# MachinePerceptionLab/Attentive_DFPrior

Measured on AMD Instinct MI355X. Metric: rendered rays/sec (64 samples/ray), Replica room0, higher is better.
Workload: dtype f32 via f16x3 split (3 f16 MFMA products per f32 product: 22-bit products, f32 accumulate); 1 GPU; room0 640x480 render_img, 64 spp (48+16), synthetic box room, seed-0 random decoders, grids at the REFERENCE init (N(0,.01), high N(0,1e-4)); stage color, ray_batch_size 100000 (per-batch far clamp, rendered as one call with a depth maximum per 100 000-ray segment), ONE frame per step; samples_per_ray=64

## Files before the change

attentive_dfprior_amd/csrc/adfp_decode_g.h:

```cpp
#pragma once
#include "adfp_decode_h.h"

__host__ __device__ constexpr int unit16(int k) { return 16 * ((k & 7) >> 2) + 4 * (k >> 3) + (k & 3); }

template <int CDIM, int NOUT>
struct DecLayoutG {
    using F = DecLayout<CDIM, NOUT>;
    static constexpr int KG_E = 3;
    static constexpr int KG_C = CDIM / 32;
    __host__ __device__ static constexpr int kg(int i) { return i == 0 ? KG_E : (i == 3 ? KG_E + 1 : 1); }
    static constexpr int P_BM = 0;
    __host__ __device__ static constexpr int layer_words(int i) { return kg(i) * 1024 + 32 + KG_C * 1024 + 32; }
    __host__ __device__ static constexpr int P_WP(int i) {
        int o = 384;
        for (int k = 0; k < i; ++k) o += layer_words(k);
        return o;
    }
    __host__ __device__ static constexpr int P_BP(int i) { return P_WP(i) + kg(i) * 1024; }
    __host__ __device__ static constexpr int P_WC(int i) { return P_BP(i) + 32; }
    __host__ __device__ static constexpr int P_BC(int i) { return P_WC(i) + KG_C * 1024; }
    static constexpr int P_WO = P_WP(5);
    static constexpr int P_BO = P_WO + NOUT * 32;
    static constexpr int P_FLAG = P_BO + 4;
    static constexpr int NFLAG = (((P_FLAG + 511) / 256) + 3) & ~3;
// ... 42 lines not shown

template <int CDIM, int NOUT>
ADFP_DEV void pack_decoder_g_block(int blk, const float* __restrict__ flat, unsigned* __restrict__ packed, int* __restrict__ status, int bit) {
    using L = DecLayoutG<CDIM, NOUT>;
    const int t = blk * 256 + (int)threadIdx.x;
    HSrc s{0, -1, -1};
    float a = 0.f, b = 0.f;
    if (t < L::P_FLAG) {
        s = dec_g_src<CDIM, NOUT>(t);
        a = s.s0 < 0 ? 0.f : flat[s.s0]; b = s.s1 < 0 ? 0.f : flat[s.s1];
    }
    pack_block_flag(!(fmaxf(fabsf(a), fabsf(b)) < 65504.0f), packed + L::P_FLAG + blk, status, bit);
    if (t >= L::P_FLAG) return;
    if (s.kind == 0) { packed[t] = s.s0 < 0 ? 0u : __float_as_uint(a); return; }
    a = f16_clamp(a); b = f16_clamp(b);
    const float ah = f16_hi_part(a), bh = f16_hi_part(b);
    _Float16 x, y;
    if (s.kind == 1) { x = (_Float16)ah; y = (_Float16)bh; }
    else { x = (_Float16)(a - ah); y = (_Float16)(b - bh); }
    packed[t] = (unsigned)__builtin_bit_cast(unsigned short, x) | ((unsigned)__builtin_bit_cast(unsigned short, y) << 16);
}
template <int CDIM, int NOUT>
__global__ void k_pack_decoder_g(const float* __restrict__ flat, unsigned* __restrict__ packed, int* __restrict__ status, int bit) { pack_decoder_g_block<CDIM, NOUT>((int)blockIdx.x, flat, packed, status, bit); }

typedef float f32x4g __attribute__((ext_vector_type(4)));

ADFP_DEV void swap_halves(float& x, float& y) {
    const auto r = __builtin_amdgcn_permlane32_swap(__float_as_uint(x), __float_as_uint(y), false, false);
    x = __uint_as_float(r[0]); y = __uint_as_float(r[1]);
}

template <int NG>
ADFP_DEV void mfma_chain_g(f32x4g acc[2][2], const unsigned* __restrict__ w, const f16x8 (*xh)[2], const f16x8 (*xl)[2]) {
#pragma unroll
    for (int kg = 0; kg < NG; ++kg) {
#pragma unroll
        for (int ob = 0; ob < 2; ++ob) {
            const f16x8 ah = __builtin_bit_cast(f16x8, *(const u32x4*)(w + kg * 1024 + ob * 512));
            const f16x8 al = __builtin_bit_cast(f16x8, *(const u32x4*)(w + kg * 1024 + ob * 512 + 256));
#pragma unroll
            for (int pb = 0; pb < 2; ++pb) {
                acc[ob][pb] = __builtin_amdgcn_mfma_f32_16x16x32_f16(ah, xh[kg][pb], acc[ob][pb], 0, 0, 0);
                acc[ob][pb] = __builtin_amdgcn_mfma_f32_16x16x32_f16(ah, xl[kg][pb], acc[ob][pb], 0, 0, 0);
                acc[ob][pb] = __builtin_amdgcn_mfma_f32_16x16x32_f16(al, xh[kg][pb], acc[ob][pb], 0, 0, 0);
            }
        }
    }
    __builtin_amdgcn_sched_barrier(0);
}

ADFP_DEV void row_store(float* p, const f32x4 v) {
    *(f32x4*)p = v;
}
template <int CDIM, int NOUT, int TRAIN = 0>
ADFP_DEV void decode_net_g(const unsigned* __restrict__ ldsu, const GridDev& grid, const GridDev& grid1, const float pn[3], const float (*pf)[3],
                           int lane, float& amax, float (*out)[NOUT], unsigned* __restrict__ mw, float* srow0, unsigned rowbits) {
    using L = DecLayoutG<CDIM, NOUT>;
    using ST = DecStage<CDIM>;
    const int g = lane >> 4;
    float* srow[2] = {nullptr, nullptr};
    if constexpr (TRAIN) {
        srow[0] = (rowbits & 1u) ? srow0 : nullptr;
        srow[1] = (rowbits & 2u) ? srow0 + 16 * ST::NXM : nullptr;
    }
    const unsigned* wl = ldsu + 4 * lane;
    const float* b4 = (const float*)ldsu + 4 * g;
    const float* brow = (const float*)ldsu + 32 * g;
    f16x8 ch[L::KG_C][2], cl[L::KG_C][2];
#pragma unroll
    for (int kc = 0; kc < L::KG_C; ++kc) {
        float c[16];
        gather16(kc == 0 ? grid : grid1, pn, g & 1, c);
        float x[8] = {c[0], c[1], c[2], c[3], c[8], c[9], c[10], c[11]};
        float y[8] = {c[4], c[5], c[6], c[7], c[12], c[13], c[14], c[15]};
#pragma unroll
        for (int s = 0; s < 8; ++s) swap_halves(x[s], y[s]);
        if constexpr (TRAIN) {
            static_assert(!TRAIN || CDIM == 32, "training rows: 32-channel decoders");
            if (srow[0]) { row_store(srow[0] + ST::xm(ST::SC) + 4 * g, f32x4{x[0], x[1], x[2], x[3]}); row_store(srow[0] + ST::xm(ST::SC) + 16 + 4 * g, f32x4{x[4], x[5], x[6], x[7]}); }
            if (srow[1]) { row_store(srow[1] + ST::xm(ST::SC) + 4 * g, f32x4{y[0], y[1], y[2], y[3]}); row_store(srow[1] + ST::xm(ST::SC) + 16 + 4 * g, f32x4{y[4], y[5], y[6], y[7]}); }
        }
        split8(x, ch[kc][0], cl[kc][0], amax);
        split8(y, ch[kc][1], cl[kc][1], amax);
    }
    f16x8 eh[L::KG_E][2], el[L::KG_E][2];
#pragma unroll
    for (int kg = 0; kg < L::KG_E; ++kg) {
        float e0[8], e1[8];
#pragma unroll
        for (int j = 0; j < 8; ++j) {
            const f32x4 bm = *(const f32x4*)(brow + L::P_BM + (32 * kg + j) * 4);
            e0[j] = adfp_sinf(fmaf(pf[0][2], bm.z, fmaf(pf[0][1], bm.y, pf[0][0] * bm.x)));
            e1[j] = adfp_sinf(fmaf(pf[1][2], bm.z, fmaf(pf[1][1], bm.y, pf[1][0] * bm.x)));
        }
        split8<false>(e0, eh[kg][0], el[kg][0], amax);
        split8<false>(e1, eh[kg][1], el[kg][1], amax);
    }
    __builtin_amdgcn_sched_barrier(0);
    f32x4g acc[2][2];
    f16x8 hh[1][2], hl[1][2];
    unsigned mk[3] = {0u, 0u, 0u};
#pragma unroll
    for (int i = 0; i < 5; ++i) {
#pragma unroll
        for (int ob = 0; ob < 2; ++ob) { const f32x4 t = *(const f32x4*)(b4 + L::P_BP(i) + 16 * ob); acc[ob][0] = t; acc[ob][1] = t; }
        if (i == 0) mfma_chain_g<L::KG_E>(acc, wl + L::P_WP(0), eh, el);
        else if (i == 3) {
            mfma_chain_g<L::KG_E>(acc, wl + L::P_WP(3), eh, el);
            mfma_chain_g<1>(acc, wl + L::P_WP(3) + L::KG_E * 1024, hh, hl);
        } else mfma_chain_g<1>(acc, wl + L::P_WP(i), hh, hl);
#pragma unroll
        for (int ob = 0; ob < 2; ++ob) {
            const f32x4 t = *(const f32x4*)(b4 + L::P_BC(i) + 16 * ob);
#pragma unroll
            for (int pb = 0; pb < 2; ++pb)
#pragma unroll
                for (int r = 0; r < 4; ++r) {
                    const float v = relu_f(acc[ob][pb][r]);
                    if constexpr (TRAIN) mk[i >> 1] = __builtin_amdgcn_alignbit(mk[i >> 1], 0u - __float_as_uint(v), 31);
                    acc[ob][pb][r] = v + t[r];
                }
        }
        mfma_chain_g<L::KG_C>(acc, wl + L::P_WC(i), ch, cl);
        if constexpr (TRAIN) {
#pragma unroll
            for (int pb = 0; pb < 2; ++pb) if (srow[pb]) {
                row_store(srow[pb] + ST::xm(ST::SH(i)) + 4 * g, f32x4{acc[0][pb][0], acc[0][pb][1], acc[0][pb][2], acc[0][pb][3]});
                row_store(srow[pb] + ST::xm(ST::SH(i)) + 16 + 4 * g, f32x4{acc[1][pb][0], acc[1][pb][1], acc[1][pb][2], acc[1][pb][3]});
            }
        }
        if (i < 4) {
#pragma unroll
            for (int pb = 0; pb < 2; ++pb) {
                const float t[8] = {acc[0][pb][0], acc[0][pb][1], acc[0][pb][2], acc[0][pb][3],
                                    acc[1][pb][0], acc[1][pb][1], acc[1][pb][2], acc[1][pb][3]};
                split8(t, hh[0][pb], hl[0][pb], amax);
            }
        }
    }
#pragma unroll
    for (int o = 0; o < NOUT; ++o) {
        const f32x4 w0 = *(const f32x4*)(b4 + L::P_WO + 32 * o), w1 = *(const f32x4*)(b4 + L::P_WO + 32 * o + 16);
#pragma unroll
        for (int pb = 0; pb < 2; ++pb) {
            float s = 0.f;
#pragma unroll
            for (int r = 0; r < 4; ++r) s = fmaf(acc[0][pb][r], w0[r], s);
#pragma unroll
            for (int r = 0; r < 4; ++r) s = fmaf(acc[1][pb][r], w1[r], s);
            s += __shfl_xor(s, 16);
            s += __shfl_xor(s, 32);
            out[pb][o] = s + ((const float*)ldsu)[L::P_BO + o];
        }
    }
    if constexpr (TRAIN) {
        const int sh = 4 * (g >> 1);
        unsigned wpb[2][3];
#pragma unroll
        for (int pb = 0; pb < 2; ++pb) {
            unsigned f[5];
#pragma unroll
            for (int i = 0; i < 5; ++i) {
                const unsigned m16 = (i == 4 || (i & 1)) ? (mk[i >> 1] & 0xFFFFu) : (mk[i >> 1] >> 16);
                const unsigned n0 = (m16 >> (12 - 4 * pb)) & 0xFu, n1 = (m16 >> (4 - 4 * pb)) & 0xFu;
                f[i] = (n0 << (12 - sh)) | (n1 << (4 - sh));
            }
            wpb[pb][0] = f[0] | (f[1] << 16); wpb[pb][1] = f[2] | (f[3] << 16); wpb[pb][2] = f[4];
        }
#pragma unroll
        for (int k = 0; k < 3; ++k) {
            const auto r = __builtin_amdgcn_permlane32_swap(wpb[0][k], wpb[1][k], false, false);
            mw[k] = r[0] | r[1];
        }
    }
}

template <int NT>
__global__ __launch_bounds__(NT, NT / 256) void k_decode_lc16(DecodeLCArgs a) {
    using LL = DecLayoutG<32, 1>;
    using LC = DecLayoutG<32, 4>;
    __shared__ __attribute__((aligned(16))) unsigned lds_all[LL::P_TOTAL + LC::P_TOTAL];
    __shared__ int s_next;
    __shared__ unsigned long long s_ring[ADFP_POOL_RING];
    unsigned* lds_low = lds_all;
    unsigned* lds_col = lds_all + LL::P_TOTAL;
    image_to_lds<NT, LL::P_TOTAL / 4>(lds_low, a.packed_low);
    image_to_lds<NT, LC::P_TOTAL / 4>(lds_col, a.packed_color);
    if (threadIdx.x == 0) s_next = NT / 64;
    if (threadIdx.x < ADFP_POOL_RING) s_ring[threadIdx.x] = 0ull;
    __syncthreads();
    const int lane = threadIdx.x & 63, n = lane & 15, g = lane >> 4;
    const int count = a.P.n;
    const int ntiles = (count + 31) >> 5;
    const TilePlan plan = tile_plan(ntiles, (int)gridDim.x, NT / 64, a.pool != nullptr);
    float amax_low = image_out_of_range<LL::P_FLAG, LL::NFLAG>(lds_low) ? INFINITY : 0.f;
    float amax_col = image_out_of_range<LC::P_FLAG, LC::NFLAG>(lds_col) ? INFINITY : 0.f;
    for (int j = threadIdx.x >> 6, tile; (tile = claim_tile_pool<NT / 64>(j, &s_next, s_ring, plan, ntiles, a.pool, a.status)) >= 0;) {
        const int idx = tile * 32 + 16 * (g >> 1) + n;
        const bool valid = idx < count;
        const int q = valid ? idx : 0;
        float pn[3], pf[2][3];
        bool pnan, keep_occ;
        {
            double pt[3];
            load_point(a.P, q, pt);
            normalize3(a.nb, pt, pn);
            const float f0 = (float)pt[0], f1 = (float)pt[1], f2 = (float)pt[2];
            pnan = (pt[0] != pt[0]) | (pt[1] != pt[1]) | (pt[2] != pt[2]);
            const unsigned f = a.flags ? a.flags[q] : 0u;
            keep_occ = (f & ADFP_F_BAND) || in_bound(pt, a.b) || !a.apply_bound;
            pf[0][0] = f0; pf[0][1] = f1; pf[0][2] = f2; pf[1][0] = f0; pf[1][1] = f1; pf[1][2] = f2;
        }
#pragma unroll
        for (int k = 0; k < 3; ++k) swap_halves(pf[0][k], pf[1][k]);
        float occ[2][1], rgb[2][4];
        int off_low = 0, off_col = LL::P_TOTAL;
        asm volatile("" : "+v"(off_low), "+v"(off_col));
        decode_net_g<32, 1>(lds_all + off_low, a.g_low, a.g_low, pn, pf, lane, amax_low, occ, nullptr, nullptr, 0u);
        asm volatile("" : "+v"(pn[0]), "+v"(pn[1]), "+v"(pn[2]), "+v"(occ[0][0]), "+v"(occ[1][0]));
        __builtin_amdgcn_sched_barrier(0);
        decode_net_g<32, 4>(lds_all + off_col, a.g_color, a.g_color, pn, pf, lane, amax_col, rgb, nullptr, nullptr, 0u);
        if (valid && (g & 1) == 0) {
            const int pb = g >> 1;
            const float nanv = __builtin_nanf("");
            const float o = pnan ? nanv : (keep_occ ? (pb ? occ[1][0] : occ[0][0]) : 100.f);
            const f32x4 c4 = pb ? f32x4{rgb[1][0], rgb[1][1], rgb[1][2], o} : f32x4{rgb[0][0], rgb[0][1], rgb[0][2], o};
            *(f32x4*)(a.raw + 4ll * q) = pnan ? f32x4{nanv, nanv, nanv, o} : c4;
            if (a.write_w) a.w[q] = 1.f;
        }
    }
    report_range(a.status, amax_low, ADFP_STATUS_F16_RANGE_LOW, a.call_flag);
    report_range(a.status, amax_col, ADFP_STATUS_F16_RANGE_COLOR, a.call_flag);
}

struct DecodeLCTrainArgs {
    DecodeLCArgs f;
    unsigned* masks_low; unsigned* masks_color;
    float* act_low; float* act_color;
    int split_networks;
};
template <int NT, bool SPLIT = false>
__global__ __launch_bounds__(NT, NT / 256) void k_decode_lc16_train(DecodeLCTrainArgs t) {
    const DecodeLCArgs& a = t.f;
    using LL = DecLayoutG<32, 1>;
    using LC = DecLayoutG<32, 4>;
    using ST = DecStage<32>;
    __shared__ __attribute__((aligned(16))) unsigned lds_all[LL::P_TOTAL + LC::P_TOTAL];
    __shared__ int s_next;
    unsigned* lds_low = lds_all;
    unsigned* lds_col = lds_all + LL::P_TOTAL;
    image_to_lds<NT, LL::P_TOTAL / 4>(lds_low, a.packed_low);
    image_to_lds<NT, LC::P_TOTAL / 4>(lds_col, a.packed_color);
    if (threadIdx.x == 0) s_next = NT / 64;
    __syncthreads();
    const int lane = threadIdx.x & 63, n = lane & 15, g = lane >> 4;
    const int count = a.P.n;
    const int ntiles = (count + 31) >> 5;
    float amax_low = image_out_of_range<LL::P_FLAG, LL::NFLAG>(lds_low) ? INFINITY : 0.f;
    float amax_col = image_out_of_range<LC::P_FLAG, LC::NFLAG>(lds_col) ? INFINITY : 0.f;
    constexpr bool split = SPLIT;
    const int njobs = split ? 2 * ntiles : ntiles;
    for (int j = threadIdx.x >> 6, job; (job = claim_tile<NT / 64>(j, &s_next, njobs)) >= 0;) {
// ... 8 lines not shown
            double pt[3];
            load_point(a.P, q, pt);
            normalize3(a.nb, pt, pn);
            pnan = (pt[0] != pt[0]) | (pt[1] != pt[1]) | (pt[2] != pt[2]);
            const float f0 = pnan ? 0.f : (float)pt[0], f1 = pnan ? 0.f : (float)pt[1], f2 = pnan ? 0.f : (float)pt[2];
            const unsigned f = a.flags ? a.flags[q] : 0u;
            keep_occ = (f & ADFP_F_BAND) || in_bound(pt, a.b) || !a.apply_bound;
            pf[0][0] = f0; pf[0][1] = f1; pf[0][2] = f2; pf[1][0] = f0; pf[1][1] = f1; pf[1][2] = f2;
        }
#pragma unroll
        for (int k = 0; k < 3; ++k) swap_halves(pf[0][k], pf[1][k]);
        const int i0 = tile * 32 + n;
        const unsigned rowbits = (i0 < count ? 1u : 0u) | (i0 + 16 < count ? 2u : 0u);
        float occ[2][1], rgb[2][4];
        unsigned mw[3];
        int off_low = 0, off_col = LL::P_TOTAL;
        asm volatile("" : "+v"(off_low), "+v"(off_col));
        if constexpr (split) {
            occ[0][0] = 0.f; occ[1][0] = 0.f;
#pragma unroll
            for (int k = 0; k < 4; ++k) { rgb[0][k] = 0.f; rgb[1][k] = 0.f; }
        }
        if (do_low) {
            decode_net_g<32, 1, 1>(lds_all + off_low, a.g_low, a.g_low, pn, pf, lane, amax_low, occ, mw, t.act_low + (long long)i0 * ST::NXM, t.act_low ? rowbits : 0u);
            if (valid) { unsigned* mrow = t.masks_low + ((long long)q * 2 + (g & 1)) * 3; mrow[0] = mw[0]; mrow[1] = mw[1]; mrow[2] = mw[2]; }
        }
        asm volatile("" : "+v"(pn[0]), "+v"(pn[1]), "+v"(pn[2]), "+v"(occ[0][0]), "+v"(occ[1][0]));
        __builtin_amdgcn_sched_barrier(0);
        if (do_col) {
            decode_net_g<32, 4, 1>(lds_all + off_col, a.g_color, a.g_color, pn, pf, lane, amax_col, rgb, mw, t.act_color + (long long)i0 * ST::NXM, t.act_color ? rowbits : 0u);
            if (valid) { unsigned* mrow = t.masks_color + ((long long)q * 2 + (g & 1)) * 3; mrow[0] = mw[0]; mrow[1] = mw[1]; mrow[2] = mw[2]; }
        }
        if (valid && (g & 1) == 0) {
            const int pb = g >> 1;
            const float nanv = __builtin_nanf("");
            const float o = pnan ? nanv : (keep_occ ? (pb ? occ[1][0] : occ[0][0]) : 100.f);
            const f32x4 c4 = pb ? f32x4{rgb[1][0], rgb[1][1], rgb[1][2], o} : f32x4{rgb[0][0], rgb[0][1], rgb[0][2], o};
            const f32x4 row = pnan ? f32x4{nanv, nanv, nanv, o} : c4;
            if (!split) {
                *(f32x4*)(a.raw + 4ll * q) = row;
                if (a.write_w) a.w[q] = 1.f;
            } else if (do_low) {
                a.raw[4ll * q + 3] = row.w;
                if (a.write_w) a.w[q] = 1.f;
            } else {
                a.raw[4ll * q] = row.x; a.raw[4ll * q + 1] = row.y; a.raw[4ll * q + 2] = row.z;
            }
        }
    }
    report_range(a.status, amax_low, ADFP_STATUS_F16_RANGE_LOW, a.call_flag);
    report_range(a.status, amax_col, ADFP_STATUS_F16_RANGE_COLOR, a.call_flag);
}

template <int NT>
__global__ __launch_bounds__(NT, NT / 256) void k_decode_high_g(DecodeArgs a) {
    using L = DecLayoutG<64, 1>;
    __shared__ __attribute__((aligned(16))) unsigned ldsu[L::P_TOTAL];
    __shared__ int s_next;
    __shared__ unsigned long long s_ring[ADFP_POOL_RING];
    image_to_lds<NT, L::P_TOTAL / 4>(ldsu, a.packed);
    if (threadIdx.x == 0) s_next = NT / 64;
    if (threadIdx.x < ADFP_POOL_RING) s_ring[threadIdx.x] = 0ull;
    __syncthreads();
    const int lane = threadIdx.x & 63, n = lane & 15, g = lane >> 4;
    const int count = *a.count_ptr;
    const int ntiles = (count + 31) >> 5;
    const TilePlan plan = tile_plan(ntiles, (int)gridDim.x, NT / 64, a.pool != nullptr);
    float amax = image_out_of_range<L::P_FLAG, L::NFLAG>(ldsu) ? INFINITY : 0.f;
    for (int j = threadIdx.x >> 6, tile; (tile = claim_tile_pool<NT / 64>(j, &s_next, s_ring, plan, ntiles, a.pool, a.status)) >= 0;) {
        const int idx = tile * 32 + 16 * (g >> 1) + n;
        const bool valid = idx < count;
        const int q = a.list[valid ? idx : 0];
        float pn[3], pf[2][3];
        bool pnan;
        const float low_occ = (a.single || !valid) ? 0.f : a.raw[4ll * q + 3];
        {
            double pt[3];
            load_point(a.P, q, pt);
            normalize3(a.nb, pt, pn);
            const float f0 = (float)pt[0], f1 = (float)pt[1], f2 = (float)pt[2];
            pnan = (pt[0] != pt[0]) | (pt[1] != pt[1]) | (pt[2] != pt[2]);
            pf[0][0] = f0; pf[0][1] = f1; pf[0][2] = f2; pf[1][0] = f0; pf[1][1] = f1; pf[1][2] = f2;
        }
#pragma unroll
        for (int k = 0; k < 3; ++k) swap_halves(pf[0][k], pf[1][k]);
        float out[2][1];
        decode_net_g<64, 1>(ldsu, a.g0, a.g1, pn, pf, lane, amax, out, nullptr, nullptr, 0u);
        if (valid && (g & 1) == 0) {
            const float o = g >> 1 ? out[1][0] : out[0][0];
            const float v = pnan ? __builtin_nanf("") : o;
            a.att_occ[idx] = a.single ? v : v + low_occ;
        }
    }
    report_range(a.status, amax, ADFP_STATUS_F16_RANGE_HIGH, a.call_flag);
}

struct AttLayoutG {
    using F = AttLayout;
    static constexpr int P_A0 = 0;
    static constexpr int P_W1 = 256;
    static constexpr int P_B1 = P_W1 + 4 * 2 * 1024;
    static constexpr int P_W2 = P_B1 + 128;
    static constexpr int P_B2 = P_W2 + 4 * 4 * 1024;
    static constexpr int P_W3 = P_B2 + 128;
    static constexpr int P_B3 = P_W3 + 2 * 4 * 1024;
    static constexpr int P_WO = P_B3 + 64;
    static constexpr int P_BO = P_WO + 128;
    static constexpr int P_FLAG = P_BO + 4;
    static constexpr int NFLAG = (((P_FLAG + 511) / 256) + 3) & ~3;
    static constexpr int P_TOTAL = P_FLAG + NFLAG;
    static_assert((P_TOTAL + 255) / 256 <= NFLAG, "one flag word per pack block");
};

__device__ HSrc att_g_src(int t) {
    using L = AttLayoutG;
    using F = AttLayout;
    if (t < L::P_W1) {
        const int row = t >> 2, c = t & 3;
        const int u = (row & ~31) + unit16(row & 31);
        return HSrc{0, c < 2 ? F::F_W0 + u * 2 + c : (c == 2 ? F::F_B0 + u : -1), -1};
    }
    auto chain = [](int u, int ngrp, int base, int ld) {
        const int blk = u / (ngrp * 1024), v = u % (ngrp * 1024);
        const int grp = v >> 10, ob = (v >> 9) & 1, part = (v >> 8) & 1, g = (v >> 6) & 3, row = 32 * blk + 16 * ob + ((v >> 2) & 15), jp = (v & 3) * 2;
        return HSrc{1 + part, base + row * ld + 32 * grp + unit16(8 * g + jp), base + row * ld + 32 * grp + unit16(8 * g + jp + 1)};
    };
    if (t < L::P_B1) return chain(t - L::P_W1, 2, F::F_W1, 64);
    if (t < L::P_W2) return HSrc{0, F::F_B1 + (t - L::P_B1), -1};
    if (t < L::P_B2) return chain(t - L::P_W2, 4, F::F_W2, 128);
    if (t < L::P_W3) return HSrc{0, F::F_B2 + (t - L::P_B2), -1};
    if (t < L::P_B3) return chain(t - L::P_W3, 4, F::F_W3, 128);
    if (t < L::P_WO) return HSrc{0, F::F_B3 + (t - L::P_B3), -1};
    if (t < L::P_BO) return HSrc{0, F::F_WO + (t - L::P_WO), -1};
    const int o = t - L::P_BO;
    return HSrc{0, o < 2 ? F::F_BO + o : -1, -1};
}

ADFP_DEV void pack_attention_g_block(int blk, const float* __restrict__ flat, unsigned* __restrict__ packed, int* __restrict__ status) {
    using L = AttLayoutG;
    const int t = blk * 256 + (int)threadIdx.x;
    HSrc s{0, -1, -1};
    float a = 0.f, b = 0.f;
    if (t < L::P_FLAG) {
        s = att_g_src(t);
// ... 125 lines not shown
```

attentive_dfprior_amd/csrc/adfp_device.h:

```cpp
#pragma once
#include <hip/hip_runtime.h>
#include <stdint.h>
#include "adfp.h"

typedef float f32x16 __attribute__((ext_vector_type(16)));
typedef float f32x4 __attribute__((ext_vector_type(4)));

#define ADFP_DEV __device__ __forceinline__

#define ADFP_F_INBOUND 1u
#define ADFP_F_BAND    2u

struct NormDev {
    double lo[3];
    double inv[3];
};

struct GridDev { const float* data; int Z, Y, X; float fZ1, fY1, fX1; };
struct TsdfDev { const float* data; int Z, Y, X; long long sZ, sY, sX; const float* cb; };

struct PtsDev {
    int mode;
    int S;
    int n;
    const void* pts;
    const float* ro;
    const float* rd;
    const double* z;
};

ADFP_DEV void load_point(const PtsDev& P, int q, double p[3]) {
    if (P.mode == ADFP_PTS_RAYS) {
        const int r = (int)((unsigned)q / (unsigned)P.S);
        const double z = P.z[q];
#pragma unroll
        for (int k = 0; k < 3; ++k)
            p[k] = __dadd_rn((double)P.ro[3 * r + k], __dmul_rn((double)P.rd[3 * r + k], z));
    } else if (P.mode == ADFP_PTS_F64) {
        const double* s = (const double*)P.pts + 3ll * q;
        p[0] = s[0]; p[1] = s[1]; p[2] = s[2];
    } else {
        const float* s = (const float*)P.pts + 3ll * q;
        p[0] = (double)s[0]; p[1] = (double)s[1]; p[2] = (double)s[2];
    }
}

ADFP_DEV bool in_bound(const double p[3], const double b[6]) {
    return (p[0] < b[1]) & (p[0] > b[0]) & (p[1] < b[3]) & (p[1] > b[2]) & (p[2] < b[5]) & (p[2] > b[4]);
}

ADFP_DEV void normalize3(const NormDev& nb, const double p[3], float pn[3]) {
#pragma unroll
    for (int k = 0; k < 3; ++k) pn[k] = (float)(((p[k] - nb.lo[k]) * nb.inv[k]) * 2.0 - 1.0);
}

ADFP_DEV void tri_axis(float pn, int size, int& i0, int& i1, float& w0, float& w1) {
    float c = ((pn + 1.f) / 2.f) * (float)(size - 1);
    c = fminf(fmaxf(c, 0.f), (float)(size - 1));
    const float f = floorf(c);
    i0 = (int)f;
    w1 = c - f;
    w0 = (f + 1.f) - c;
    i1 = i0 + 1;
    if (i1 > size - 1) { i1 = size - 1; w1 = 0.f; }
}

typedef float f32x2_u __attribute__((ext_vector_type(2), aligned(4)));
ADFP_DEV float trilerp_scalar(const TsdfDev& t, const float pn[3]) {
    int x0, x1, y0, y1, z0, z1; float wx0, wx1, wy0, wy1, wz0, wz1;
    tri_axis(pn[0], t.X, x0, x1, wx0, wx1);
    tri_axis(pn[1], t.Y, y0, y1, wy0, wy1);
    tri_axis(pn[2], t.Z, z0, z1, wz0, wz1);
    const float* d = t.data;
    const long long ox0 = x0 * t.sX, ox1 = x1 * t.sX, oy0 = y0 * t.sY, oy1 = y1 * t.sY;
    float v000, v001, v010, v011, v100, v101, v110, v111;
    if (t.sZ == 1 && t.Z >= 2) {
        const int zb = z0 < t.Z - 1 ? z0 : t.Z - 2;
        const bool lo = z0 == zb;
        const f32x2_u p00 = *(const f32x2_u*)(d + zb + oy0 + ox0);
        const f32x2_u p01 = *(const f32x2_u*)(d + zb + oy0 + ox1);
        const f32x2_u p10 = *(const f32x2_u*)(d + zb + oy1 + ox0);
        const f32x2_u p11 = *(const f32x2_u*)(d + zb + oy1 + ox1);
        v000 = lo ? p00.x : p00.y; v100 = p00.y;
        v001 = lo ? p01.x : p01.y; v101 = p01.y;
        v010 = lo ? p10.x : p10.y; v110 = p10.y;
        v011 = lo ? p11.x : p11.y; v111 = p11.y;
    } else {
        const long long oz0 = z0 * t.sZ, oz1 = z1 * t.sZ;
        v000 = d[oz0 + oy0 + ox0]; v001 = d[oz0 + oy0 + ox1];
        v010 = d[oz0 + oy1 + ox0]; v011 = d[oz0 + oy1 + ox1];
// ... 411 lines not shown
```

attentive_dfprior_amd/csrc/adfp_kernels.hip:

```cpp
#include "adfp_device.h"
#include <math.h>
#include <string.h>
#include <stdio.h>
#include <stdlib.h>

#define ADFP_CHECK_LAUNCH()                         \
    do {                                            \
        hipError_t e_ = hipGetLastError();          \
        if (e_ != hipSuccess) return (int)e_;       \
    } while (0)

__global__ __launch_bounds__(256) void k_zero(unsigned* __restrict__ p, long long n_words) {
    const long long n4 = n_words >> 2;
    const long long stride = (long long)gridDim.x * 256;
    if ((((unsigned long long)p) & 15ull) == 0) {
        for (long long i = (long long)blockIdx.x * 256 + threadIdx.x; i < n4; i += stride) ((uint4*)p)[i] = uint4{0u, 0u, 0u, 0u};
        for (long long i = (n4 << 2) + (long long)blockIdx.x * 256 + threadIdx.x; i < n_words; i += stride) p[i] = 0u;
    } else {
        for (long long i = (long long)blockIdx.x * 256 + threadIdx.x; i < n_words; i += stride) p[i] = 0u;
    }
}
#define ZERO_MULTI 8
struct ZeroJobs { unsigned* p[ZERO_MULTI]; long long words[ZERO_MULTI]; unsigned first_block[ZERO_MULTI + 1]; int n; };
__device__ inline void zero_multi_block(const ZeroJobs& z, unsigned blk) {
// ... 1579 lines not shown
    PtsDev P; int rc = make_pts(pts, &P); if (rc) return rc;
    adfp_scene sc; memset(&sc, 0, sizeof(sc));
    sc.tsdf = *tsdf;
    for (int k = 0; k < 3; ++k) { sc.tsdf_bnds[k][0] = tsdf_bnds[k][0]; sc.tsdf_bnds[k][1] = tsdf_bnds[k][1]; sc.bound[k][0] = 0; sc.bound[k][1] = 1; }
    return launch_tsdf(&sc, P, nullptr, nullptr, nullptr, nullptr, nullptr, out, (hipStream_t)stream);
}

static int decode_grid(int ntiles, int waves_per_wg, int wg_per_cu) {
    int g = (ntiles + waves_per_wg - 1) / waves_per_wg;
    const int cap = num_cu() * wg_per_cu;
    if (g > cap) g = cap;
    return g < 1 ? 1 : g;
}

static int eval_points_impl(const adfp_scene* sc, const PtsDev& P, int stage, int apply_bound, float* raw, float* w, Workspace& ws_in, hipStream_t st,
                            const adfp_train_state* state = nullptr, bool ws_counter_is_zero = false) {
    if (P.n == 0) return 0;
    Workspace ws = ws_in;
    if (state) {
        ws.flags = state->flags; ws.list = state->list; ws.counter = state->counter;
        ws.att_occ = state->att_occ; ws.att_u = state->att_u;
    }
    hipError_t e;
    const bool fuse = stage != ADFP_STAGE_LOW;
    if (stage != ADFP_STAGE_COLOR) {
        e = zero_async(raw, (size_t)P.n * 16, st);
        if (e != hipSuccess) return (int)e;
    }
    const bool any_h = sc->h_low || (fuse && (sc->h_high || sc->h_att)) || (stage == ADFP_STAGE_COLOR && sc->h_color);
    int* call_flag = (any_h && ws.counter) ? ws.counter + 8 : nullptr;
    if ((fuse || any_h || state) && ws.counter && !ws_counter_is_zero) {
        e = zero_async(ws.counter, 64, st);
        if (e != hipSuccess) return (int)e;
    }
    if (fuse) {
        int rc = launch_tsdf(sc, P, ws.flags, ws.list, ws.att_u, nullptr, ws.counter, nullptr, st);
        if (rc) return rc;
    }
    DecodeArgs a;
    a.P = P; a.nb = make_norm(sc->bound); fill_bound(a.b, sc->bound);
    a.list = nullptr; a.count_ptr = nullptr; a.flags = fuse ? ws.flags : nullptr;
    a.raw = raw; a.w = w; a.att_occ = nullptr; a.write_w = 1; a.apply_bound = apply_bound;
    a.status = sc->status; a.masks = nullptr; a.act = nullptr; a.single = 0; a.call_flag = call_flag;
    const int ntiles = (P.n + 31) / 32;
    const bool fused_lc = stage == ADFP_STAGE_COLOR && !state && sc->h_low && sc->h_color;
    if (fused_lc) {
        DecodeLCArgs f;
        f.P = P; f.nb = a.nb; fill_bound(f.b, sc->bound);
        f.g_low = make_grid(sc->low); f.g_color = make_grid(sc->color);
        f.packed_low = (const unsigned*)sc->h_low; f.packed_color = (const unsigned*)sc->h_color;
        f.flags = a.flags; f.raw = raw; f.w = w; f.write_w = 1; f.apply_bound = apply_bound; f.status = sc->status; f.call_flag = call_flag;
        f.pool = ws.counter ? ws.counter + 10 : nullptr;
        f.packed_low += DecLayoutH<32, 1>::P_TOTAL; f.packed_color += DecLayoutH<32, 4>::P_TOTAL;
        hipLaunchKernelGGL((k_decode_lc16<ADFP_LC_NT>), dim3(decode_grid(ntiles, ADFP_LC_NT / 64, 1)), dim3(ADFP_LC_NT), 0, st, f);
        ADFP_CHECK_LAUNCH();
    }
    const bool fused_lc_train = stage == ADFP_STAGE_COLOR && state && sc->h_low && sc->h_color && state->masks_low && state->masks_color;
    if (fused_lc_train) {
        DecodeLCTrainArgs t;
        DecodeLCArgs& f = t.f;
        f.P = P; f.nb = a.nb; fill_bound(f.b, sc->bound);
        f.g_low = make_grid(sc->low); f.g_color = make_grid(sc->color);
        f.packed_low = (const unsigned*)sc->h_low + DecLayoutH<32, 1>::P_TOTAL; f.packed_color = (const unsigned*)sc->h_color + DecLayoutH<32, 4>::P_TOTAL;
        f.flags = a.flags; f.raw = raw; f.w = w; f.write_w = 1; f.apply_bound = apply_bound; f.status = sc->status; f.call_flag = call_flag; f.pool = nullptr;
        t.masks_low = state->masks_low; t.masks_color = state->masks_color; t.act_low = state->act_low; t.act_color = state->act_color;
        t.split_networks = 2 * ntiles <= num_cu() * (ADFP_LCT_NT / 64) ? 1 : 0;
        if (t.split_networks) hipLaunchKernelGGL((k_decode_lc16_train<ADFP_LCT_NT, true>), dim3(decode_grid(2 * ntiles, ADFP_LCT_NT / 64, 1)), dim3(ADFP_LCT_NT), 0, st, t);
        else hipLaunchKernelGGL((k_decode_lc16_train<ADFP_LCT_NT, false>), dim3(decode_grid(ntiles, ADFP_LCT_NT / 64, 1)), dim3(ADFP_LCT_NT), 0, st, t);
        ADFP_CHECK_LAUNCH();
    }
    a.g0 = make_grid(sc->low); a.g1 = a.g0;
    if (fused_lc || fused_lc_train) {
    } else if (sc->h_low && state && state->masks_low) {
        a.packed = (const float*)sc->h_low; a.masks = state->masks_low; a.act = state->act_low;
        if (a.act) hipLaunchKernelGGL((k_decode_h<32, 1, ROLE_LOW, 512, 2>), dim3(decode_grid(ntiles, 8, 1)), dim3(512), 0, st, a);
        else hipLaunchKernelGGL((k_decode_h<32, 1, ROLE_LOW, 512, 1>), dim3(decode_grid(ntiles, 8, 1)), dim3(512), 0, st, a);
        a.masks = nullptr; a.act = nullptr;
    } else if (sc->h_low) {
        a.packed = (const float*)sc->h_low;
            hipLaunchKernelGGL((k_decode_h<32, 1, ROLE_LOW, ADFP_DECH_NT>), dim3(decode_grid(ntiles, ADFP_DECH_NT / 64, ADFP_DECH_WG)), dim3(ADFP_DECH_NT), 0, st, a);
    } else {
        a.packed = sc->w_low;
        hipLaunchKernelGGL((k_decode<32, 1, ROLE_LOW, 256>), dim3(decode_grid(ntiles, 4, 2)), dim3(256), 0, st, a);
    }
    ADFP_CHECK_LAUNCH();
    if (stage == ADFP_STAGE_COLOR && !fused_lc && !fused_lc_train) {
        a.g0 = make_grid(sc->color); a.g1 = a.g0;
        if (sc->h_color && state && state->masks_color) {
            a.packed = (const float*)sc->h_color; a.masks = state->masks_color; a.act = state->act_color;
            if (a.act) hipLaunchKernelGGL((k_decode_h<32, 4, ROLE_COLOR, 512, 2>), dim3(decode_grid(ntiles, 8, 1)), dim3(512), 0, st, a);
            else hipLaunchKernelGGL((k_decode_h<32, 4, ROLE_COLOR, 512, 1>), dim3(decode_grid(ntiles, 8, 1)), dim3(512), 0, st, a);
            a.masks = nullptr; a.act = nullptr;
        } else if (sc->h_color) {
            a.packed = (const float*)sc->h_color;
            hipLaunchKernelGGL((k_decode_h<32, 4, ROLE_COLOR, ADFP_DECH_NT>), dim3(decode_grid(ntiles, ADFP_DECH_NT / 64, ADFP_DECH_WG)), dim3(ADFP_DECH_NT), 0, st, a);
        } else {
            a.packed = sc->w_color;
            hipLaunchKernelGGL((k_decode<32, 4, ROLE_COLOR, 256>), dim3(decode_grid(ntiles, 4, 2)), dim3(256), 0, st, a);
        }
        ADFP_CHECK_LAUNCH();
    }
    if (fuse) {
        a.g0 = make_grid(sc->high); a.g1 = make_grid(sc->low);
        a.list = ws.list; a.count_ptr = ws.counter; a.att_occ = ws.att_occ;
        if (sc->h_high && state && state->masks_high) {
            a.packed = (const float*)sc->h_high; a.masks = state->masks_high; a.act = state->act_high;
            if (a.act) hipLaunchKernelGGL((k_decode_h<64, 1, ROLE_HIGH, 512, 2>), dim3(decode_grid(ntiles, 8, 1)), dim3(512), 0, st, a);
            else hipLaunchKernelGGL((k_decode_h<64, 1, ROLE_HIGH, 512, 1>), dim3(decode_grid(ntiles, 8, 1)), dim3(512), 0, st, a);
            a.masks = nullptr; a.act = nullptr;
        } else if (sc->h_high) {
            a.packed = (const float*)((const unsigned*)sc->h_high + DecLayoutH<64, 1>::P_TOTAL);
            a.pool = ws.counter ? ws.counter + 11 : nullptr;
            hipLaunchKernelGGL((k_decode_high_g<ADFP_HIGH_NT>), dim3(decode_grid(ntiles, ADFP_HIGH_NT / 64, 1)), dim3(ADFP_HIGH_NT), 0, st, a);
        } else {
            a.packed = sc->w_high;
            hipLaunchKernelGGL((k_decode<64, 1, ROLE_HIGH, 512>), dim3(decode_grid(ntiles, 8, 1)), dim3(512), 0, st, a);
        }
        ADFP_CHECK_LAUNCH();
        AttArgs t;
        t.list = ws.list; t.count_ptr = ws.counter; t.att_occ = ws.att_occ; t.att_u = ws.att_u;
        t.flags = ws.flags; t.raw = raw; t.w = w; t.apply_bound = apply_bound; t.status = sc->status; t.n_rows = 0; t.call_flag = call_flag;
        t.masks = nullptr; t.act = nullptr;
        if (sc->h_att && state && state->masks_att) {
            t.packed = (const float*)sc->h_att; t.masks = state->masks_att; t.act = state->act_att;
            hipLaunchKernelGGL((k_attention_h<1, 256>), dim3(decode_grid(ntiles, 4, 1)), dim3(256), 0, st, t);
        } else if (sc->h_att) {
            t.packed = (const float*)((const unsigned*)sc->h_att + AttLayoutH::P_TOTAL);
            t.pool = ws.counter ? ws.counter + 12 : nullptr;
            hipLaunchKernelGGL(k_attention_g<512>, dim3(decode_grid(ntiles, 8, 1)), dim3(512), 0, st, t);
        } else {
            t.packed = sc->w_att;
            hipLaunchKernelGGL(k_attention, dim3(decode_grid(ntiles, 8, 1)), dim3(512), 0, st, t);
        }
        ADFP_CHECK_LAUNCH();
    }
    if (call_flag && sc->flat_low && (!fuse || (sc->flat_high && sc->flat_att)) && (stage != ADFP_STAGE_COLOR || sc->flat_color)) {
        FallbackArgs f;
        f.P = P; f.nb = a.nb; fill_bound(f.b, sc->bound);
        f.low = make_grid(sc->low); f.high = make_grid(sc->high); f.color = make_grid(sc->color);
        f.flat_low = sc->flat_low; f.flat_high = sc->flat_high; f.flat_color = sc->flat_color; f.flat_att = sc->flat_att;
        f.stage = stage; f.apply_bound = apply_bound;
        f.flags = fuse ? ws.flags : nullptr; f.list = ws.list; f.count_ptr = ws.counter; f.att_u = ws.att_u; f.att_occ = ws.att_occ;
        f.raw = raw; f.w = w; f.call_flag = call_flag;
        long long blocks = ((long long)P.n * (fuse ? 2 : 1) + 255) / 256;
        const long long cap = (long long)num_cu() * 8;
        hipLaunchKernelGGL(k_fallback_points, dim3((unsigned)(blocks < cap ? blocks : cap)), dim3(256), 0, st, f);
        ADFP_CHECK_LAUNCH();
    }
    return 0;
}

extern "C" int adfp_decode_stage(const adfp_scene* sc, const adfp_points* pts, int kind, float* raw, float* w, int* tile_counter, void* stream) {
    if (!sc || !pts || !raw || !w) return ADFP_E_ARG;
    if (kind != ADFP_DEC_LOW && kind != ADFP_DEC_COLOR && kind != ADFP_DEC_LOW_COLOR) return ADFP_E_UNSUPPORTED;
    if (grid_too_big(sc->low) || grid_too_big(sc->color)) return ADFP_E_UNSUPPORTED;
    PtsDev P; int rc = make_pts(pts, &P); if (rc) return rc;
    if (P.n == 0) return 0;
    if (kind == ADFP_DEC_LOW_COLOR) {
        if (!sc->low.data || !sc->color.data || !sc->h_low || !sc->h_color) return ADFP_E_ARG;
        DecodeLCArgs f;
        f.P = P; f.nb = make_norm(sc->bound); fill_bound(f.b, sc->bound);
        f.g_low = make_grid(sc->low); f.g_color = make_grid(sc->color);
        f.packed_low = (const unsigned*)sc->h_low; f.packed_color = (const unsigned*)sc->h_color;
        f.flags = nullptr; f.raw = raw; f.w = w; f.write_w = 1; f.apply_bound = 1; f.status = sc->status; f.call_flag = nullptr; f.pool = tile_counter;
        if (tile_counter) { hipError_t e = zero_async(tile_counter, 4, (hipStream_t)stream); if (e != hipSuccess) return (int)e; }
        f.packed_low += DecLayoutH<32, 1>::P_TOTAL; f.packed_color += DecLayoutH<32, 4>::P_TOTAL;
        hipLaunchKernelGGL((k_decode_lc16<ADFP_LC_NT>), dim3(decode_grid((P.n + 31) / 32, ADFP_LC_NT / 64, 1)), dim3(ADFP_LC_NT), 0, (hipStream_t)stream, f);
        ADFP_CHECK_LAUNCH();
        return 0;
    }
    DecodeArgs a;
    a.P = P; a.nb = make_norm(sc->bound); fill_bound(a.b, sc->bound);
    a.list = nullptr; a.count_ptr = nullptr; a.flags = nullptr;
    a.raw = raw; a.w = w; a.att_occ = nullptr; a.write_w = 1; a.apply_bound = 1; a.status = sc->status;
    a.masks = nullptr; a.act = nullptr; a.single = 0; a.call_flag = nullptr;
    const int ntiles = (P.n + 31) / 32;
    hipStream_t st = (hipStream_t)stream;
    if (kind == ADFP_DEC_LOW) {
        if (!sc->low.data || !(sc->w_low || sc->h_low)) return ADFP_E_ARG;
        a.g0 = make_grid(sc->low); a.g1 = a.g0;
        if (sc->h_low) {
            a.packed = (const float*)sc->h_low;
            hipLaunchKernelGGL((k_decode_h<32, 1, ROLE_LOW, ADFP_DECH_NT>), dim3(decode_grid(ntiles, ADFP_DECH_NT / 64, ADFP_DECH_WG)), dim3(ADFP_DECH_NT), 0, st, a);
        } else {
            a.packed = sc->w_low;
            hipLaunchKernelGGL((k_decode<32, 1, ROLE_LOW, 256>), dim3(decode_grid(ntiles, 4, 2)), dim3(256), 0, st, a);
        }
    } else {
        if (!sc->color.data || !(sc->w_color || sc->h_color)) return ADFP_E_ARG;
        a.g0 = make_grid(sc->color); a.g1 = a.g0;
        if (sc->h_color) {
            a.packed = (const float*)sc->h_color;
            hipLaunchKernelGGL((k_decode_h<32, 4, ROLE_COLOR, ADFP_DECH_NT>), dim3(decode_grid(ntiles, ADFP_DECH_NT / 64, ADFP_DECH_WG)), dim3(ADFP_DECH_NT), 0, st, a);
        } else {
            a.packed = sc->w_color;
            hipLaunchKernelGGL((k_decode<32, 4, ROLE_COLOR, 256>), dim3(decode_grid(ntiles, 4, 2)), dim3(256), 0, st, a);
        }
    }
    ADFP_CHECK_LAUNCH();
    return 0;
}

__global__ __launch_bounds__(256) void k_inv_tsdf(const float* __restrict__ t, float* __restrict__ u, long long n) {
    const long long i = (long long)blockIdx.x * 256 + threadIdx.x;
    if (i < n) u[i] = inv_tsdf(t[i]);
}
extern "C" int adfp_decode_single(const adfp_scene* sc, const adfp_points* pts, int kind, float* out4, void* stream) {
    if (!sc || !pts || !out4) return ADFP_E_ARG;
    if (grid_too_big(sc->low) || grid_too_big(sc->high) || grid_too_big(sc->color)) return ADFP_E_UNSUPPORTED;
    PtsDev P; int rc = make_pts(pts, &P); if (rc) return rc;
    if (P.n == 0) return 0;
    DecodeArgs a;
    a.P = P; a.nb = make_norm(sc->bound); fill_bound(a.b, sc->bound);
    a.list = nullptr; a.count_ptr = nullptr; a.flags = nullptr;
    a.raw = out4; a.w = nullptr; a.att_occ = nullptr; a.write_w = 0; a.apply_bound = 0; a.status = sc->status;
    a.masks = nullptr; a.act = nullptr; a.single = 1; a.call_flag = nullptr;
    const int ntiles = (P.n + 31) / 32;
    hipStream_t st = (hipStream_t)stream;
    if (kind == ADFP_DEC_LOW) {
        if (!sc->low.data || !(sc->w_low || sc->h_low)) return ADFP_E_ARG;
// ... 1265 lines not shown
```

Before: 59.11 million rays/s.

## Prefetch next tile's ray point loads during decode in ray-mode decoder kernels

Adds RAYS-specialised variants of the low/color and high decode kernels. In the high kernel, the next tile is claimed early and its ray origin, direction, depth and low-occupancy loads are issued through a hook placed after the grid gather, so their latency overlaps the MLP work of the current tile. In the low/color kernel, the flag load is issued together with the point loads ahead of the double-precision point computation. This hides global-load latency at the cost of more live registers and a more complex tile-claim loop.

```diff
diff --git a/attentive_dfprior_amd/csrc/adfp_decode_g.h b/attentive_dfprior_amd/csrc/adfp_decode_g.h
--- a/attentive_dfprior_amd/csrc/adfp_decode_g.h
+++ b/attentive_dfprior_amd/csrc/adfp_decode_g.h
@@ -118,9 +118,11 @@
 ADFP_DEV void row_store(float* p, const f32x4 v) {
     *(f32x4*)p = v;
 }
-template <int CDIM, int NOUT, int TRAIN = 0>
+struct NoHook { ADFP_DEV void operator()() const {} };
+template <int CDIM, int NOUT, int TRAIN = 0, typename HOOK = NoHook>
 ADFP_DEV void decode_net_g(const unsigned* __restrict__ ldsu, const GridDev& grid, const GridDev& grid1, const float pn[3], const float (*pf)[3],
-                           int lane, float& amax, float (*out)[NOUT], unsigned* __restrict__ mw, float* srow0, unsigned rowbits) {
+                           int lane, float& amax, float (*out)[NOUT], unsigned* __restrict__ mw, float* srow0, unsigned rowbits,
+                           const HOOK& after_gather = HOOK()) {
     using L = DecLayoutG<CDIM, NOUT>;
     using ST = DecStage<CDIM>;
     const int g = lane >> 4;
@@ -149,6 +151,7 @@
         split8(x, ch[kc][0], cl[kc][0], amax);
         split8(y, ch[kc][1], cl[kc][1], amax);
     }
+    after_gather();
     f16x8 eh[L::KG_E][2], el[L::KG_E][2];
 #pragma unroll
     for (int kg = 0; kg < L::KG_E; ++kg) {
@@ -241,7 +244,7 @@
     }
 }
 
-template <int NT>
+template <int NT, bool RAYS>
 __global__ __launch_bounds__(NT, NT / 256) void k_decode_lc16(DecodeLCArgs a) {
     using LL = DecLayoutG<32, 1>;
     using LC = DecLayoutG<32, 4>;
@@ -269,11 +272,22 @@
         bool pnan, keep_occ;
         {
             double pt[3];
-            load_point(a.P, q, pt);
+            unsigned f;
+            if constexpr (RAYS) {
+                RayFront fr;
+                ray_point_issue(a.P, q, fr);
+                const unsigned char* fp = a.flags ? a.flags + q : (const unsigned char*)(a.P.z + q);
+                const unsigned fb = *fp;
+                __builtin_amdgcn_sched_barrier(0);
+                ray_point_finish(fr, pt);
+                f = a.flags ? fb : 0u;
+            } else {
+                load_point(a.P, q, pt);
+                f = a.flags ? a.flags[q] : 0u;
+            }
             normalize3(a.nb, pt, pn);
             const float f0 = (float)pt[0], f1 = (float)pt[1], f2 = (float)pt[2];
             pnan = (pt[0] != pt[0]) | (pt[1] != pt[1]) | (pt[2] != pt[2]);
-            const unsigned f = a.flags ? a.flags[q] : 0u;
             keep_occ = (f & ADFP_F_BAND) || in_bound(pt, a.b) || !a.apply_bound;
             pf[0][0] = f0; pf[0][1] = f1; pf[0][2] = f2; pf[1][0] = f0; pf[1][1] = f1; pf[1][2] = f2;
         }
@@ -388,7 +402,7 @@
     report_range(a.status, amax_col, ADFP_STATUS_F16_RANGE_COLOR, a.call_flag);
 }
 
-template <int NT>
+template <int NT, bool RAYS>
 __global__ __launch_bounds__(NT, NT / 256) void k_decode_high_g(DecodeArgs a) {
     using L = DecLayoutG<64, 1>;
     __shared__ __attribute__((aligned(16))) unsigned ldsu[L::P_TOTAL];
@@ -403,29 +417,74 @@
     const int ntiles = (count + 31) >> 5;
     const TilePlan plan = tile_plan(ntiles, (int)gridDim.x, NT / 64, a.pool != nullptr);
     float amax = image_out_of_range<L::P_FLAG, L::NFLAG>(ldsu) ? INFINITY : 0.f;
-    for (int j = threadIdx.x >> 6, tile; (tile = claim_tile_pool<NT / 64>(j, &s_next, s_ring, plan, ntiles, a.pool, a.status)) >= 0;) {
-        const int idx = tile * 32 + 16 * (g >> 1) + n;
-        const bool valid = idx < count;
-        const int q = a.list[valid ? idx : 0];
-        float pn[3], pf[2][3];
-        bool pnan;
-        const float low_occ = (a.single || !valid) ? 0.f : a.raw[4ll * q + 3];
-        {
-            double pt[3];
-            load_point(a.P, q, pt);
-            normalize3(a.nb, pt, pn);
-            const float f0 = (float)pt[0], f1 = (float)pt[1], f2 = (float)pt[2];
-            pnan = (pt[0] != pt[0]) | (pt[1] != pt[1]) | (pt[2] != pt[2]);
-            pf[0][0] = f0; pf[0][1] = f1; pf[0][2] = f2; pf[1][0] = f0; pf[1][1] = f1; pf[1][2] = f2;
-        }
-#pragma unroll
-        for (int k = 0; k < 3; ++k) swap_halves(pf[0][k], pf[1][k]);
-        float out[2][1];
-        decode_net_g<64, 1>(ldsu, a.g0, a.g1, pn, pf, lane, amax, out, nullptr, nullptr, 0u);
-        if (valid && (g & 1) == 0) {
-            const float o = g >> 1 ? out[1][0] : out[0][0];
-            const float v = pnan ? __builtin_nanf("") : o;
-            a.att_occ[idx] = a.single ? v : v + low_occ;
+    if constexpr (RAYS) {
+        const int lp = 16 * (g >> 1) + n;
+        int j = threadIdx.x >> 6;
+        int tile = claim_tile_pool<NT / 64>(j, &s_next, s_ring, plan, ntiles, a.pool, a.status);
+        RayFront fr;
+        float low_next = 0.f;
+        auto issue_front = [&](int q) {
+            ray_point_issue(a.P, q, fr);
+            const float* lo = a.single ? (const float*)(a.P.z + q) : a.raw + (4ll * q + 3);
+            low_next = *lo;
+        };
+        if (tile >= 0) {
+            const int idx = tile * 32 + lp;
+            issue_front(a.list[idx < count ? idx : 0]);
+        }
+        while (tile >= 0) {
+            const int idx = tile * 32 + lp;
+            const bool valid = idx < count;
+            const int tile_n = claim_tile_pool<NT / 64>(j, &s_next, s_ring, plan, ntiles, a.pool, a.status);
+            const int idx_n = tile_n * 32 + lp;
+            const int q_n = a.list[(tile_n >= 0 && idx_n < count) ? idx_n : 0];
+            float pn[3], pf[2][3];
+            bool pnan;
+            const float low_occ = a.single ? 0.f : low_next;
+            {
+                double pt[3];
+                ray_point_finish(fr, pt);
+                normalize3(a.nb, pt, pn);
+                const float f0 = (float)pt[0], f1 = (float)pt[1], f2 = (float)pt[2];
+                pnan = (pt[0] != pt[0]) | (pt[1] != pt[1]) | (pt[2] != pt[2]);
+                pf[0][0] = f0; pf[0][1] = f1; pf[0][2] = f2; pf[1][0] = f0; pf[1][1] = f1; pf[1][2] = f2;
+            }
+#pragma unroll
+            for (int k = 0; k < 3; ++k) swap_halves(pf[0][k], pf[1][k]);
+            float out[2][1];
+            decode_net_g<64, 1, 0>(ldsu, a.g0, a.g1, pn, pf, lane, amax, out, nullptr, nullptr, 0u, [&]() { issue_front(q_n); });
+            if (valid && (g & 1) == 0) {
+                const float o = g >> 1 ? out[1][0] : out[0][0];
+                const float v = pnan ? __builtin_nanf("") : o;
+                a.att_occ[idx] = a.single ? v : v + low_occ;
+            }
+            tile = tile_n;
+        }
+    } else {
+        for (int j = threadIdx.x >> 6, tile; (tile = claim_tile_pool<NT / 64>(j, &s_next, s_ring, plan, ntiles, a.pool, a.status)) >= 0;) {
+            const int idx = tile * 32 + 16 * (g >> 1) + n;
+            const bool valid = idx < count;
+            const int q = a.list[valid ? idx : 0];
+            float pn[3], pf[2][3];
+            bool pnan;
+            const float low_occ = (a.single || !valid) ? 0.f : a.raw[4ll * q + 3];
+            {
+                double pt[3];
+                load_point(a.P, q, pt);
+                normalize3(a.nb, pt, pn);
+                const float f0 = (float)pt[0], f1 = (float)pt[1], f2 = (float)pt[2];
+                pnan = (pt[0] != pt[0]) | (pt[1] != pt[1]) | (pt[2] != pt[2]);
+                pf[0][0] = f0; pf[0][1] = f1; pf[0][2] = f2; pf[1][0] = f0; pf[1][1] = f1; pf[1][2] = f2;
+            }
+#pragma unroll
+            for (int k = 0; k < 3; ++k) swap_halves(pf[0][k], pf[1][k]);
+            float out[2][1];
+            decode_net_g<64, 1>(ldsu, a.g0, a.g1, pn, pf, lane, amax, out, nullptr, nullptr, 0u);
+            if (valid && (g & 1) == 0) {
+                const float o = g >> 1 ? out[1][0] : out[0][0];
+                const float v = pnan ? __builtin_nanf("") : o;
+                a.att_occ[idx] = a.single ? v : v + low_occ;
+            }
         }
     }
     report_range(a.status, amax, ADFP_STATUS_F16_RANGE_HIGH, a.call_flag);
diff --git a/attentive_dfprior_amd/csrc/adfp_device.h b/attentive_dfprior_amd/csrc/adfp_device.h
--- a/attentive_dfprior_amd/csrc/adfp_device.h
+++ b/attentive_dfprior_amd/csrc/adfp_device.h
@@ -29,13 +29,22 @@
     const double* z;
 };
 
+struct RayFront { double z; float ro[3], rd[3]; };
+ADFP_DEV void ray_point_issue(const PtsDev& P, int q, RayFront& f) {
+    const int r = (int)((unsigned)q / (unsigned)P.S);
+    f.z = P.z[q];
+#pragma unroll
+    for (int k = 0; k < 3; ++k) { f.ro[k] = P.ro[3 * r + k]; f.rd[k] = P.rd[3 * r + k]; }
+}
+ADFP_DEV void ray_point_finish(const RayFront& f, double p[3]) {
+#pragma unroll
+    for (int k = 0; k < 3; ++k) p[k] = __dadd_rn((double)f.ro[k], __dmul_rn((double)f.rd[k], f.z));
+}
 ADFP_DEV void load_point(const PtsDev& P, int q, double p[3]) {
     if (P.mode == ADFP_PTS_RAYS) {
-        const int r = (int)((unsigned)q / (unsigned)P.S);
-        const double z = P.z[q];
-#pragma unroll
-        for (int k = 0; k < 3; ++k)
-            p[k] = __dadd_rn((double)P.ro[3 * r + k], __dmul_rn((double)P.rd[3 * r + k], z));
+        RayFront f;
+        ray_point_issue(P, q, f);
+        ray_point_finish(f, p);
     } else if (P.mode == ADFP_PTS_F64) {
         const double* s = (const double*)P.pts + 3ll * q;
         p[0] = s[0]; p[1] = s[1]; p[2] = s[2];
diff --git a/attentive_dfprior_amd/csrc/adfp_kernels.hip b/attentive_dfprior_amd/csrc/adfp_kernels.hip
--- a/attentive_dfprior_amd/csrc/adfp_kernels.hip
+++ b/attentive_dfprior_amd/csrc/adfp_kernels.hip
@@ -1655,7 +1655,8 @@
         f.flags = a.flags; f.raw = raw; f.w = w; f.write_w = 1; f.apply_bound = apply_bound; f.status = sc->status; f.call_flag = call_flag;
         f.pool = ws.counter ? ws.counter + 10 : nullptr;
         f.packed_low += DecLayoutH<32, 1>::P_TOTAL; f.packed_color += DecLayoutH<32, 4>::P_TOTAL;
-        hipLaunchKernelGGL((k_decode_lc16<ADFP_LC_NT>), dim3(decode_grid(ntiles, ADFP_LC_NT / 64, 1)), dim3(ADFP_LC_NT), 0, st, f);
+        if (P.mode == ADFP_PTS_RAYS) hipLaunchKernelGGL((k_decode_lc16<ADFP_LC_NT, true>), dim3(decode_grid(ntiles, ADFP_LC_NT / 64, 1)), dim3(ADFP_LC_NT), 0, st, f);
+        else hipLaunchKernelGGL((k_decode_lc16<ADFP_LC_NT, false>), dim3(decode_grid(ntiles, ADFP_LC_NT / 64, 1)), dim3(ADFP_LC_NT), 0, st, f);
         ADFP_CHECK_LAUNCH();
     }
     const bool fused_lc_train = stage == ADFP_STAGE_COLOR && state && sc->h_low && sc->h_color && state->masks_low && state->masks_color;
@@ -1714,7 +1715,8 @@
         } else if (sc->h_high) {
             a.packed = (const float*)((const unsigned*)sc->h_high + DecLayoutH<64, 1>::P_TOTAL);
             a.pool = ws.counter ? ws.counter + 11 : nullptr;
-            hipLaunchKernelGGL((k_decode_high_g<ADFP_HIGH_NT>), dim3(decode_grid(ntiles, ADFP_HIGH_NT / 64, 1)), dim3(ADFP_HIGH_NT), 0, st, a);
+            if (P.mode == ADFP_PTS_RAYS) hipLaunchKernelGGL((k_decode_high_g<ADFP_HIGH_NT, true>), dim3(decode_grid(ntiles, ADFP_HIGH_NT / 64, 1)), dim3(ADFP_HIGH_NT), 0, st, a);
+            else hipLaunchKernelGGL((k_decode_high_g<ADFP_HIGH_NT, false>), dim3(decode_grid(ntiles, ADFP_HIGH_NT / 64, 1)), dim3(ADFP_HIGH_NT), 0, st, a);
         } else {
             a.packed = sc->w_high;
             hipLaunchKernelGGL((k_decode<64, 1, ROLE_HIGH, 512>), dim3(decode_grid(ntiles, 8, 1)), dim3(512), 0, st, a);
@@ -1768,7 +1770,8 @@
         f.flags = nullptr; f.raw = raw; f.w = w; f.write_w = 1; f.apply_bound = 1; f.status = sc->status; f.call_flag = nullptr; f.pool = tile_counter;
         if (tile_counter) { hipError_t e = zero_async(tile_counter, 4, (hipStream_t)stream); if (e != hipSuccess) return (int)e; }
         f.packed_low += DecLayoutH<32, 1>::P_TOTAL; f.packed_color += DecLayoutH<32, 4>::P_TOTAL;
-        hipLaunchKernelGGL((k_decode_lc16<ADFP_LC_NT>), dim3(decode_grid((P.n + 31) / 32, ADFP_LC_NT / 64, 1)), dim3(ADFP_LC_NT), 0, (hipStream_t)stream, f);
+        if (P.mode == ADFP_PTS_RAYS) hipLaunchKernelGGL((k_decode_lc16<ADFP_LC_NT, true>), dim3(decode_grid((P.n + 31) / 32, ADFP_LC_NT / 64, 1)), dim3(ADFP_LC_NT), 0, (hipStream_t)stream, f);
+        else hipLaunchKernelGGL((k_decode_lc16<ADFP_LC_NT, false>), dim3(decode_grid((P.n + 31) / 32, ADFP_LC_NT / 64, 1)), dim3(ADFP_LC_NT), 0, (hipStream_t)stream, f);
         ADFP_CHECK_LAUNCH();
         return 0;
     }
```

Result: faster. 59.75 million rays/s (median of 6 runs) (+1.1%).
